# Veason-silverbullet/DIGAT

Measured on AMD Instinct MI355X. Metric: MIND dev impressions scored/sec (AUC match not run), higher is better.
Workload: dtype f32; 1 GPU; MIND-small default: --graph_encoder=DIGAT neighbors=3 hops=2 (N=10, U=67), d=400, graph_depth=3, fp32 dev inference; projection=auto -> fp16x3, N=10, U=67, d=400, graph_depth=3, news_num=65238, parallelism=dp1 (row shards, no data-path collective), ranks_in_process_group=1

## Files before the change

digat_amd/csrc/digat_glue.inc:

```

__global__ void __launch_bounds__(256) build_user_nodes_kernel(const float4* ue, const float4* topic, float4* Xu,
                                                               long B, int H, int C, int d4, const int* group, const uint8_t* rowmask = nullptr) {
    const long per_row = (long)(H + C) * d4;
    const long total = B * per_row;
    for (long i = (long)blockIdx.x * 256 + threadIdx.x; i < total; i += (long)gridDim.x * 256) {
        const long b = i / per_row;
        if (rowmask && rowmask[b] == 0) continue;
        const long rem = i - b * per_row;
        const long hist = (long)H * d4;
        const long src = group ? group[b] : b;
        Xu[i] = rem < hist ? ue[src * hist + rem] : topic[rem - hist];
    }
}

struct UserNodes3 { const float4* hist[3]; const float4* topic[3]; float4* dst[3]; };
__global__ void __launch_bounds__(256) build_user_nodes3_kernel(const UserNodes3 a, long B, int H, int C, int d4) {
    const int pl = blockIdx.y;
    const float4* ue = a.hist[pl];
    const float4* topic = a.topic[pl];
    float4* Xu = a.dst[pl];
    const long per_row = (long)(H + C) * d4;
    const long total = B * per_row;
    const long hist = (long)H * d4;
    for (long i = (long)blockIdx.x * 256 + threadIdx.x; i < total; i += (long)gridDim.x * 256) {
        const long b = i / per_row;
        const long rem = i - b * per_row;
        Xu[i] = rem < hist ? ue[b * hist + rem] : topic[rem - hist];
    }
}

__global__ void __launch_bounds__(256) user_live_flags_kernel(const uint8_t* Au, const uint8_t* cat_mask, const int64_t* cat_idx,
                                                              int B, int U, int H, int C1, uint8_t* flags, int* cnt, int* entries,
                                                              int* hlast, uint8_t* bflags, int* bcnt,
                                                              unsigned* twin = nullptr, uint8_t* tflags = nullptr, int* tcnt = nullptr,
                                                              const uint8_t* rowmask = nullptr) {
    extern __shared__ __attribute__((aligned(16))) unsigned char live_smem[];
    const int lane = threadIdx.x & 63, wave = threadIdx.x >> 6;
    const int b = blockIdx.x * 4 + wave;
    if (b >= B) return;
    if (rowmask && rowmask[b] == 0) return;
    const int uu = U * U;
    unsigned char* Al = live_smem + wave * ((uu + 63) & ~63);
    {
        const uint8_t* Ag = Au + (long)b * uu;
        for (int k0 = 0; k0 < uu; k0 += 64 * 32) {
            uint8_t v[32];
#pragma unroll
            for (int k = 0; k < 32; ++k) v[k] = Ag[min(k0 + k * 64 + lane, uu - 1)];
#pragma unroll
            for (int k = 0; k < 32; ++k) if (k0 + k * 64 + lane < uu) Al[k0 + k * 64 + lane] = v[k];
// ... 45 lines not shown
            if (i < H) {
                const long c = cat_idx[(long)b * H + i];
                live |= !any_cat || (c >= 0 && c < C1 && cat_mask[(long)b * C1 + c] != 0);
            }
            flags[(long)b * U + i] = live ? 1 : 0;
        }
        lv2[h] = live;
        count += __popcll(__ballot(live));
        const unsigned long long hm = __ballot(live && i < H);
        if (hm) last = 64 * h + 64 - __builtin_clzll(hm);
    }
    if (lane == 0) cnt[b] = count;
    if (lane == 0 && hlast) hlast[b] = last;
    if (twin) {
        int before[2] = {0, 0};
        unsigned word[2] = {0xFFFFFF00u | (unsigned)lane, 0xFFFFFF00u | (unsigned)(lane + 64)};
        unsigned long long rem0 = __ballot(lv2[0]), rem1 = __ballot(lv2[1]);
        while (rem0 | rem1) {
            const int hj = rem0 ? 0 : 1, lj = rem0 ? __builtin_ctzll(rem0) : __builtin_ctzll(rem1);
            const unsigned lo0 = (unsigned)__builtin_amdgcn_readlane((int)(unsigned)(hj ? own0[1] : own0[0]), lj);
            const unsigned hi0 = (unsigned)__builtin_amdgcn_readlane((int)(unsigned)((hj ? own0[1] : own0[0]) >> 32), lj);
            const unsigned lo1 = (unsigned)__builtin_amdgcn_readlane((int)(unsigned)(hj ? own1[1] : own1[0]), lj);
            const unsigned hi1 = (unsigned)__builtin_amdgcn_readlane((int)(unsigned)((hj ? own1[1] : own1[0]) >> 32), lj);
            const unsigned long long r0 = ((unsigned long long)hi0 << 32) | lo0, r1 = ((unsigned long long)hi1 << 32) | lo1;
            const bool e0 = lv2[0] && own0[0] == r0 && own1[0] == r1, e1 = lv2[1] && own0[1] == r0 && own1[1] == r1;
            const unsigned long long g0 = __ballot(e0), g1 = __ballot(e1);
            const unsigned long long below = (1ull << lane) - 1ull, above = lane == 63 ? 0ull : ~((2ull << lane) - 1ull);
            if (e0) {
                before[0] = __popcll(g0 & below);
                unsigned long long a0 = g0 & above, a1 = g1;
#pragma unroll
                for (int k = 1; k < TWIN_R; ++k) {
                    int j = -1;
                    if (a0) { j = __builtin_ctzll(a0); a0 &= a0 - 1ull; }
                    else if (a1) { j = 64 + __builtin_ctzll(a1); a1 &= a1 - 1ull; }
                    if (j >= 0) word[0] = (word[0] & ~(0xFFu << (8 * k))) | ((unsigned)j << (8 * k));
                }
            }
            if (e1) {
                before[1] = __popcll(g0) + __popcll(g1 & below);
                unsigned long long a1 = g1 & above;
#pragma unroll
                for (int k = 1; k < TWIN_R; ++k) {
                    if (a1) { const int j = 64 + __builtin_ctzll(a1); a1 &= a1 - 1ull; word[1] = (word[1] & ~(0xFFu << (8 * k))) | ((unsigned)j << (8 * k)); }
                }
            }
            rem0 &= ~g0; rem1 &= ~g1;
        }
        int leads = 0;
#pragma unroll
        for (int h = 0; h < 2; ++h) {
            const int i = lane + 64 * h;
            const bool lead = lv2[h] && (before[h] % TWIN_R) == 0;
            if (i < U) {
                twin[(long)b * U + i] = lead ? word[h] : 0xFFFFFFFFu;
                tflags[(long)b * U + i] = lead ? 1 : 0;
            }
            leads += __popcll(__ballot(lead));
        }
        if (lane == 0) tcnt[b] = leads;
    }
    if (entries && lane == 0) entries[b] = nz + (all_live ? U : 0);
    if (bflags) {
        int bc = 0;
        for (int c0 = 0; c0 < C1; c0 += 64) {
            const int c = c0 + lane;
            const bool bl = c < C1 && (!any_cat || cat_mask[(long)b * C1 + c] != 0);
            if (c < C1) bflags[(long)b * C1 + c] = bl ? 1 : 0;
            bc += __popcll(__ballot(bl));
        }
        if (lane == 0) bcnt[b] = bc;
    }
}

struct LiveExpand {
    const uint8_t* flags_g; const unsigned* twin_g; const uint8_t* tflags_g; const uint8_t* bflags_g;
    const int* cnt_g; const int* entries_g; const int* hlast_g; const int* bcnt_g; const int* tcnt_g;
    uint8_t* flags; unsigned* twin; uint8_t* tflags; uint8_t* bflags;
    int* cnt; int* entries; int* hlast; int* bcnt; int* tcnt;
};
__global__ void __launch_bounds__(256) live_expand_kernel(const LiveExpand a, const int* row_group, int B, int U, int C1) {
    const int lane = threadIdx.x & 63, wave = threadIdx.x >> 6;
    const int b = blockIdx.x * 4 + wave;
    if (b >= B) return;
    const long g = __builtin_amdgcn_readfirstlane(row_group[b]);
    if (a.flags_g == a.flags && g == b) return;
    for (int i = lane; i < U; i += 64) {
        a.flags[(long)b * U + i] = a.flags_g[g * U + i];
        if (a.twin) { a.twin[(long)b * U + i] = a.twin_g[g * U + i]; a.tflags[(long)b * U + i] = a.tflags_g[g * U + i]; }
    }
    if (a.bflags) for (int c = lane; c < C1; c += 64) a.bflags[(long)b * C1 + c] = a.bflags_g[g * C1 + c];
    if (lane == 0) {
        a.cnt[b] = a.cnt_g[g];
        if (a.hlast) a.hlast[b] = a.hlast_g[g];
        if (a.bcnt) a.bcnt[b] = a.bcnt_g[g];
        if (a.tcnt) a.tcnt[b] = a.tcnt_g[g];
        if (a.entries) a.entries[b] = a.entries_g[g];
    }
}

__global__ void __launch_bounds__(1024) sparse_decide_kernel(const int* entries, int B, int n, int per_node, int* flag) {
    __shared__ long long part[16];
    long long s = 0;
    for (int b = threadIdx.x; b < B; b += 1024) s += entries[b];
    for (int o = 32; o > 0; o >>= 1) s += __shfl_xor(s, o, 64);
    if ((threadIdx.x & 63) == 0) part[threadIdx.x >> 6] = s;
    __syncthreads();
    if (threadIdx.x == 0) {
        long long tot = 0;
        for (int w = 0; w < 16; ++w) tot += part[w];
        *flag = tot <= (long long)per_node * B * n ? 1 : 0;
// ... 286 lines not shown
```

digat_amd/csrc/digat_kernels.hip:

```cpp
#include <hip/hip_runtime.h>
#include <stdint.h>
#include <string.h>
#include <stdlib.h>
#include <atomic>
#include <initializer_list>
#include <mutex>
#include <unordered_map>
#include <utility>

#include "../../include/digat_hip.h"

typedef float v4f __attribute__((ext_vector_type(4)));

#define DIGAT_CHECK_LAUNCH()                                   \
    do {                                                       \
        if (hipGetLastError() != hipSuccess) return DIGAT_ERR_LAUNCH; \
    } while (0)

static inline size_t align_up(size_t v, size_t a) { return (v + a - 1) / a * a; }
struct Arena {
    char* base; size_t cap, used; bool ok;
    Arena() : base(nullptr), cap(SIZE_MAX), used(0), ok(true) {}
    Arena(void* p, size_t n) : base((char*)p), cap(n), used(0), ok(p != nullptr) {}
    template <class T> T* take(size_t count) {
// ... 119 lines not shown
__device__ __forceinline__ float leaky02_uniform(float e) {
    const float t = 0.2f * e;
    float r;
    asm("v_max_f32 %0, %1, %2" : "=v"(r) : "s"(e), "v"(t));
    return r;
}
__device__ __forceinline__ unsigned hash32(unsigned x) {
    x ^= x >> 16; x *= 0x7feb352dU; x ^= x >> 15; x *= 0x846ca68bU; x ^= x >> 16;
    return x;
}
__host__ __device__ __forceinline__ unsigned drop_threshold(float p) { return (unsigned)(p * 4294967296.0); }
__device__ __forceinline__ bool drop_keep(unsigned seed, long e, unsigned thr) {
    return hash32((unsigned)e * 0x9E3779B9U + hash32(seed + (unsigned)(e >> 32))) >= thr;
}
constexpr int TWIN_R = DIGAT_TWIN_R;
#include "digat_gemm.inc"
#include "digat_xattn.inc"
#include "digat_context.inc"
#include "digat_ctxfused.inc"
#include "digat_glue.inc"

extern "C" {

int digat_version(void) { return DIGAT_ABI_VERSION; }

const char* digat_error_string(int code) {
    switch (code) {
        case DIGAT_OK: return "ok";
        case DIGAT_ERR_ARG: return "bad argument (null pointer or negative size)";
        case DIGAT_ERR_SHAPE: return "unsupported shape (d % 4 != 0, graph larger than DIGAT_MAX_NODES, depth too large)";
// ... 17 lines not shown
    w.h = a.take<float>(3 * nd);
    if (w.h) { w.P = w.h + nd; w.Q = w.P + nd; }
    w.r = a.take<float>((size_t)B * d);
    w.alpha = a.take<float>((size_t)B * n * n);
    return w;
}
size_t digat_xattn_workspace_bytes(int B, int n, int d) { Arena a; xattn_carve(a, B, n, d); return a.used; }

int digat_xattn_pairwise_fwd(const float* Pr, const float* Q, const float* h, const float* X,
                             const float* a, const uint8_t* A, float* out, float* alpha,
                             int B, int n, int d, void* stream) {
    if (!Pr || !Q || !h || !X || !a || !A || !out || !alpha) return DIGAT_ERR_ARG;
    return launch_xattn_pairwise(Pr, Q, h, X, a, A, out, alpha, B, n, d, (hipStream_t)stream);
}

struct TwinLists { const unsigned* word; const int* list; const int* count; };

struct XattnOpts {
    const void* wsplit = nullptr;
    const int* rowidx = nullptr; const int* nrows_dev = nullptr; const uint8_t* live = nullptr;
    int sparse_mode = DIGAT_XATTN_DENSE; const int* sparse_flag = nullptr;
    int pq_x3 = 0, pq_mode = 0, centre_limit = 0, gemm_format = 0, prof_part = 0;
    unsigned* range_flag = nullptr; const TwinLists* tw = nullptr;
};

static int xattn_core(const float* X, const uint8_t* A, const float* r_given,
                      const float* W, const float* bW, const float* F1, const float* F2, const float* a,
                      float* out, float* alpha_out, int B, int n, int d, void* workspace, size_t workspace_bytes, hipStream_t st,
                      const XattnOpts& o = XattnOpts()) {
    Arena ar(workspace, workspace_bytes);
    const XattnWs w = xattn_carve(ar, B, n, d);
// ... 15 lines not shown
                     d / 4 <= 256 && d % 80 == 0 && (long)B * n >= 2048;
    const long ld8 = (long)align_up((size_t)d + 4 * (size_t)(d / 80), 64);
    if (pq16) { g.bf16_segs = 6; if (pq_mode & 2) g.x1_segs = 6; }
    if (pq8) { g.fp8_segs = 6; g.ldy8 = ld8; if (pq_mode & 2) g.x1_segs = 6; }
    const bool listed = rowidx && gemm_takes_row_list(g);
    if (listed) { g.rowidx = rowidx; g.nrows_dev = nrows_dev; }
    const int rc = launch_gemm(g, st, DIGAT_KERNEL_PROJ);
    if (rc) return rc;
    const int* skip_if = nullptr;
    if (sparse_mode != DIGAT_XATTN_DENSE && !alpha_out && n > 16 && d / 4 <= 256) {
        SparseArgs sg{P, Q, h, X, a, A, out, nullptr, nullptr, listed ? live : nullptr,
                      sparse_mode == DIGAT_XATTN_AUTO ? o.sparse_flag : nullptr, B, n, d / 4, 0, nullptr, nullptr,
                      listed && live ? rowidx : nullptr, listed && live ? nrows_dev : nullptr, 0, nullptr, pq8 ? 2 : (pq16 ? 1 : 0), o.centre_limit};
        sg.ld8 = pq8 ? ld8 : 0;
        sg.prof_part = o.prof_part;
        if (o.tw && listed && live) { sg.twin = o.tw->word; sg.twlist = o.tw->list; sg.twcount = o.tw->count; }
        const int rcs = launch_sparse(sg, st);
        if (rcs || sparse_mode == DIGAT_XATTN_SPARSE) return rcs;
        skip_if = o.sparse_flag;
    }
    return launch_xattn_pairwise(P, Q, h, X, a, A, out, alpha, B, n, d, st, listed ? live : nullptr, nullptr, nullptr,
                                 alpha_out != nullptr, skip_if);
}

static int xattn_fwd_k3(const float* X, const uint8_t* A, const float* ctx, const float* W, const float* bW, const float* F1,
                        const float* F2, const float* F3, const float* b3, const float* a, float* out, float* alpha_out,
                        int B, int n, int d, void* workspace, size_t workspace_bytes, void* stream, const XattnOpts& o = XattnOpts()) {
    Arena ar(workspace, workspace_bytes);
    const XattnWs w = xattn_carve(ar, B, n, d);
    if (!ar.ok) return DIGAT_ERR_WORKSPACE;
    if (B == 0) return DIGAT_OK;
// ... 324 lines not shown
struct FoldCtxWs { float *T, *T2, *glob; };
struct EncoderWs {
    float *Xu[2], *Xn[2];
    char* xws; size_t xws_bytes;
    XattnWs xu;
    char* cws; size_t cws_bytes;
    FoldCtxWs fc;
    float *kq_t, *kq_u, *r_user[2], *r_news;
    char* xws_news; size_t xws_news_bytes;
    XattnWs xn;
    int *cnt, *off, *idx, *cnt2, *off2, *idx2, *entries, *flag, *hlast;
    uint8_t *flags1, *flags2;
    int *cnt_n, *off_n, *idx_n; uint8_t* flags_n;
    int *l0_gs, *l0_off; uint8_t* l0_lead; int* l0_idx;
    unsigned* tw_word; int* tw_list; uint8_t* tw_flags; int *tw_cnt, *tw_off;
    int *gl_off, *gl_idx;
    int* idx32;
    uint8_t *Au, *cm; int64_t* ci;
    uint8_t *fg, *tfg; unsigned* twg; uint8_t* bfg; int *cg, *eg, *hg, *bcg, *tcg;
    uint8_t *same, *is_leader, *lead; int* leader_of;
};
static bool encoder_carve(Arena& a, int B, int N, int H, int C, int d, int variant, EncoderWs& e) {
    const int U = H + C, C1 = C + 1, nmax = N > U ? N : U;
    const size_t b = (size_t)B, bd = b * d, bu = b * U;
    e = EncoderWs();
    for (float*& x : e.Xu) x = a.take<float>(bu * d);
    for (float*& x : e.Xn) x = a.take<float>(b * N * d);
    Arena xa = a.sub(digat_xattn_workspace_bytes(B, nmax, d));
    e.xws = xa.base; e.xws_bytes = xa.cap;
    e.xu = xattn_carve(xa, B, U, d);
    Arena ca = a.sub(max_sz(digat_news_ctx_workspace_bytes(B, N, d), digat_user_ctx_workspace_bytes(B, U, H, C1, d)));
    e.cws = ca.base; e.cws_bytes = ca.cap;
    e.fc = FoldCtxWs{ca.take<float>(b * C1 * d), ca.take<float>(b * C1 * d), ca.take<float>(bd)};
    e.kq_t = a.take<float>(bd); e.kq_u = a.take<float>(bd);
// ... 6 lines not shown
    e.entries = a.take<int>(b); e.flag = a.take<int>(64); e.hlast = a.take<int>(b);
    e.flags1 = a.take<uint8_t>(bu); e.flags2 = a.take<uint8_t>(b * C1);
    e.cnt_n = a.take<int>(b); e.off_n = a.take<int>(b + 1); e.idx_n = a.take<int>(b * N); e.flags_n = a.take<uint8_t>(b * N);
    e.l0_gs = a.take<int>(b + 64); e.l0_off = a.take<int>(b + 64); e.l0_lead = a.take<uint8_t>(b); e.l0_idx = a.take<int>(bu);
    e.tw_word = a.take<unsigned>(bu); e.tw_list = a.take<int>(bu); e.tw_flags = a.take<uint8_t>(bu);
    e.tw_cnt = a.take<int>(b + 64); e.tw_off = a.take<int>(b + 64);
    e.gl_off = a.take<int>(b + 64); e.gl_idx = a.take<int>(bu);
    e.idx32 = a.take<int>(b);
    if (variant == ENC_GROUPED) {
        const size_t g = b / 4 + 1;
        e.Au = a.take<uint8_t>(bu * U); e.cm = a.take<uint8_t>(b * C1); e.ci = a.take<int64_t>(b * H);
        e.fg = a.take<uint8_t>(g * U); e.tfg = a.take<uint8_t>(g * U); e.twg = a.take<unsigned>(g * U); e.bfg = a.take<uint8_t>(g * C1);
        for (int** x : {&e.cg, &e.eg, &e.hg, &e.bcg, &e.tcg}) *x = a.take<int>(g);
    } else if (variant == ENC_SHARED) {
        e.same = a.take<uint8_t>(b); e.is_leader = a.take<uint8_t>(b); e.lead = a.take<uint8_t>(b); e.leader_of = a.take<int>(b);
    }
    return a.ok && xa.ok && ca.ok && na.ok;
}
static size_t encoder_ws_bytes(int B, int N, int H, int C, int d, int variant) { Arena a; EncoderWs e; encoder_carve(a, B, N, H, C, d, variant, e); return a.used; }

struct EncoderCall {
    const digat_params* p;
    const float* Xn_in; const uint8_t *An, *Mn;
    const float* ue;
    const uint8_t *Au, *cat_mask; const int64_t* cat_idx;
    const float* c_n0; float *out_news, *out_user;
    int B, N, H;
    void* workspace; size_t workspace_bytes; hipStream_t st;
    int variant;
    const int* row_group; int G;
// ... 106 lines not shown
    const int pq_mode = ((p->flags & DIGAT_PQ_BF16) ? 1 : 0) | ((p->flags & DIGAT_PQ_X1) ? 2 : 0) | ((p->flags & DIGAT_PQ_FP8) ? 4 : 0);
    const bool want_scan = want_live || sparse_mode == DIGAT_XATTN_AUTO;
    const int* rowidx = nullptr;
    const int* nrows_dev = nullptr;
    uint8_t* live_flags = nullptr;
    const int *pend_rowidx = nullptr, *pend_nrows = nullptr, *pend_bidx = nullptr, *pend_nb = nullptr, *pend_hlast = nullptr;

    uint8_t* pend_flags = nullptr;
    const bool l0_chunked = row_group && (Xg0 || shared) && want_live &&
                            sparse_mode == DIGAT_XATTN_SPARSE && d / 4 <= 128 && U <= 128;
    const uint8_t* const l0_lead = shared ? run_lead : w.l0_lead;
    const bool twins = want_live && sparse_mode == DIGAT_XATTN_SPARSE && d / 4 <= 128 && U <= 128 && L > 1;
    unsigned* const tw_word = w.tw_word; uint8_t* const tw_flags = w.tw_flags;
    int *const tw_list = w.tw_list, *const tw_cnt = w.tw_cnt, *const tw_off = w.tw_off;
    int *const gl_off = w.gl_off, *const gl_idx = w.gl_idx, *const l0_gs = w.l0_gs, *const l0_off = w.l0_off, *const l0_idx = w.l0_idx;
    TwinLists tw_pub{nullptr, nullptr, nullptr};
    auto find_live_rows = [&](hipStream_t sq) -> int {
        int *cnt = w.cnt, *off = w.off, *idx = w.idx, *cnt2 = w.cnt2, *off2 = w.off2, *idx2 = w.idx2, *entries = w.entries, *flag = w.flag;
        int* hlast = w.hlast; uint8_t *flags1 = w.flags1, *flags2 = w.flags2;
        ProfScope prof(DIGAT_KERNEL_GLUE, (double)B * ((double)U * U + 2.0 * C1 + H * 8.0) + (double)B * (U + C1) * 6, sq);
        if (l0_chunked && !shared) {
            hipLaunchKernelGGL(sparse_l0_chunks_kernel, dim3(1), dim3(1024), 0, sq, row_group, B, G, SPARSE_L0_ROWS, l0_gs, w.l0_lead);
            DIGAT_CHECK_LAUNCH();
        }
        if (shared) {
            const bool want_entries = sparse_mode == DIGAT_XATTN_AUTO;
            hipLaunchKernelGGL(user_live_flags_kernel, dim3((B + 3) / 4), dim3(256), (size_t)4 * ((U * U + 63) & ~63), sq, Au, cat_mask, cat_idx, B, U, H, C1,
                               flags1, cnt, want_entries ? entries : (int*)nullptr, hlast, flags2, cnt2,
                               twins ? tw_word : (unsigned*)nullptr, twins ? tw_flags : (uint8_t*)nullptr, twins ? tw_cnt : (int*)nullptr,
                               run_leader);
            DIGAT_CHECK_LAUNCH();
            const LiveExpand le{flags1, twins ? tw_word : nullptr, tw_flags, flags2, cnt, entries, hlast, cnt2, tw_cnt,
                                flags1, twins ? tw_word : nullptr, tw_flags, flags2,
                                cnt, want_entries ? entries : nullptr, hlast, cnt2, twins ? tw_cnt : nullptr};
            hipLaunchKernelGGL(live_expand_kernel, dim3((B + 3) / 4), dim3(256), 0, sq, le, row_group, B, U, C1);
            DIGAT_CHECK_LAUNCH();
        } else if (c.variant == ENC_GROUPED) {
            uint8_t *fg = w.fg, *tfg = w.tfg, *bfg = w.bfg; unsigned* twg = w.twg;
            int *cg = w.cg, *eg = w.eg, *hg = w.hg, *bcg = w.bcg, *tcg = w.tcg;
            const bool want_entries = sparse_mode == DIGAT_XATTN_AUTO;
            hipLaunchKernelGGL(user_live_flags_kernel, dim3((G + 3) / 4), dim3(256), (size_t)4 * ((U * U + 63) & ~63), sq, c.Au_g, c.cm_g, c.ci_g, G, U, H, C1,
                               fg, cg, want_entries ? eg : (int*)nullptr, hg, bfg, bcg,
                               twins ? twg : (unsigned*)nullptr, twins ? tfg : (uint8_t*)nullptr, twins ? tcg : (int*)nullptr);
            DIGAT_CHECK_LAUNCH();
            const LiveExpand le{fg, twins ? twg : nullptr, tfg, bfg, cg, eg, hg, bcg, tcg,
                                flags1, twins ? tw_word : nullptr, tw_flags, flags2,
                                cnt, want_entries ? entries : nullptr, hlast, cnt2, twins ? tw_cnt : nullptr};
            hipLaunchKernelGGL(live_expand_kernel, dim3((B + 3) / 4), dim3(256), 0, sq, le, row_group, B, U, C1);
            DIGAT_CHECK_LAUNCH();
        } else {
            hipLaunchKernelGGL(user_live_flags_kernel, dim3((B + 3) / 4), dim3(256), (size_t)4 * ((U * U + 63) & ~63), sq, Au, cat_mask, cat_idx, B, U, H, C1,
                               flags1, cnt, sparse_mode == DIGAT_XATTN_AUTO ? entries : (int*)nullptr, hlast, flags2, cnt2,
                               twins ? tw_word : (unsigned*)nullptr, twins ? tw_flags : (uint8_t*)nullptr, twins ? tw_cnt : (int*)nullptr);
            DIGAT_CHECK_LAUNCH();
        }
        if (sparse_mode == DIGAT_XATTN_AUTO) {
            hipLaunchKernelGGL(sparse_decide_kernel, dim3(1), dim3(1024), 0, sq, (const int*)entries, B, U, SPARSE_PER_NODE, flag);
            DIGAT_CHECK_LAUNCH();
            sparse_flag = flag;
        }
        ScanPair sp{{cnt, cnt2}, {off, off2}, {nullptr, nullptr}};
        ListPair lp{{flags1, flags2}, {off, off2}, {U, C1, U, U, U, U}, {idx, idx2}, {nullptr, nullptr}};
        int jobs = 2;
        if (l0_chunked) {
            sp.cnt[jobs] = cnt; sp.off[jobs] = l0_off; sp.rowmask[jobs] = l0_lead;
            lp.flags[jobs] = flags1; lp.off[jobs] = l0_off; lp.out[jobs] = l0_idx; lp.rowmask[jobs] = l0_lead;
            ++jobs;
        }
        if (twins) {
            sp.cnt[jobs] = tw_cnt; sp.off[jobs] = tw_off;
            lp.flags[jobs] = tw_flags; lp.off[jobs] = tw_off; lp.out[jobs] = tw_list;
            lp.width[jobs] = U;
            ++jobs;
        }
        if (shared) {
            sp.cnt[jobs] = cnt; sp.off[jobs] = gl_off; sp.rowmask[jobs] = run_leader;
            lp.flags[jobs] = flags1; lp.off[jobs] = gl_off; lp.out[jobs] = gl_idx; lp.rowmask[jobs] = run_leader;
            lp.width[jobs] = U;
            ++jobs;
        }
        hipLaunchKernelGGL(exclusive_scan2_kernel, dim3(jobs), dim3(1024), 0, sq, sp, B);
        DIGAT_CHECK_LAUNCH();
        hipLaunchKernelGGL(live_list2_kernel, dim3((B + 3) / 4, jobs), dim3(256), 0, sq, lp, B);
        DIGAT_CHECK_LAUNCH();
        pend_rowidx = idx; pend_nrows = off + B; pend_bidx = idx2; pend_nb = off2 + B; pend_flags = flags1; pend_hlast = hlast;
        return DIGAT_OK;
    };
    auto publish_live_rows = [&]() {
        rowidx = pend_rowidx; nrows_dev = pend_nrows; bucket_idx = pend_bidx; nbuckets_dev = pend_nb; live_flags = pend_flags;
        hist_last = pend_hlast;
        if (twins) tw_pub = TwinLists{tw_word, tw_list, tw_off + B};
    };
    const int side_mode = (p->flags & DIGAT_PARAMS_SIDE_STREAM_OFF) ? 0 : ((p->flags & DIGAT_PARAMS_SIDE_STREAM_ON) ? 1 : 2);
    SideStream* side = (side_mode == 0 || (side_mode == 2 && B >= 2048)) ? nullptr : side_stream(st);
    const bool news_early = L > 0 && N <= 16 && d / 4 <= 256;
    const bool news_lists_on = L > 0 && d / 4 <= 256 && !(p->flags & DIGAT_PARAMS_NO_LIVE_ROWS);
    const bool news_lists = news_lists_on && ((!news_early && (p->flags & DIGAT_NEWS_XATTN_SPARSE) && N > 16) || (news_early && L > 1 && B >= 2048));
    const int* news_rowidx = nullptr; const int* news_nrows = nullptr; const uint8_t* news_flags = nullptr;
    auto news_project = [&](int layer, const float* Xn_cur, hipStream_t sq) -> int {
        const digat_layer_params& ln = p->news[layer];
        GemmArgs gp = gemm_plain(Xn_cur, d, ln.W, ln.bW, w.xn.h, d, B * N, d, d, 0);
        gp.w[1] = ln.F1; gp.bias[1] = nullptr; gp.y[1] = w.xn.P;
        gp.w[2] = ln.F2; gp.bias[2] = nullptr; gp.y[2] = w.xn.Q;
        gp.nsegs = 3;
        gp.x3_segs = pq_x3 ? 6 : 0;
        gp.m_dispatch = 1 << 30;
// ... 556 lines not shown
```

digat_amd/csrc/digat_xattn.inc:

```

struct ScoreArgs {
    const float* P;
    const float* Q; const float* a; const uint8_t* A; float* alpha;
    float* s_out;
    const uint8_t* live;
    const int* qgroup;
    const float* radd;
    const int64_t* bindex;
    const float* agg_h; const float* agg_x; float* agg_out;
    int B, n, d, d4;
    int NT, SN, CC4, nchunks, RB;
    int img_slots;
    int ring_slots;
    int ninstr;
    int am_off;
    int a_off;
    int tl_off;
    int ld_off;
    int pm_off;
    const int* skip_if;
    uint8_t* amask; float* adrop; float drop_p; unsigned drop_seed;
};
constexpr int XA_RING = 3;
constexpr int XA_KMAX = 4;
// ... 452 lines not shown
    const int* run_if;
    int B, n, d4;
    int xgroup;
    const uint8_t* fill_flags; float* fill_out;
    const int* rowidx; const int* nrows_dev;
    int G;
    unsigned long long* exec_rows;
    int pq16;
    int centre_limit;
    int xcd_group;
    long ld8;
    const unsigned* twin; const int* twlist; const int* twcount;
    unsigned exec_unit;
    int prof_part;
    float* t_alpha; float* t_spre; uint8_t* t_amask; float t_p; unsigned t_seed;
#ifdef DIGAT_SPARSE_TIMERS
    unsigned long long* timers;
#endif
};

#ifdef DIGAT_SPARSE_TIMERS
#define SP_T0() unsigned long long sp_last = __builtin_amdgcn_s_memtime(); const bool sp_on = g.timers && (blockIdx.x & 15) == 0
#define SP_T(k) do { if (sp_on) { asm volatile("s_waitcnt vmcnt(0) lgkmcnt(0)" ::: "memory"); const unsigned long long t__ = __builtin_amdgcn_s_memtime(); \
                     if (lane == 0) atomicAdd(g.timers + (k), t__ - sp_last); sp_last = __builtin_amdgcn_s_memtime(); } } while (0)
#else
#define SP_T0() do {} while (0)
#define SP_T(k) do {} while (0)
#endif

#ifndef DIGAT_SPARSE_NBR
// ... 723 lines not shown
    uint8_t ab0 = g.A[rho * n + min(lane, n - 1)], ab1 = g.A[rho * n + min(lane + 64, n - 1)];
    int rho_next_v = g.twlist[min(k + stride, count - 1)];
    for (;;) {
        const long kn = k + stride;
        const bool more = kn < count;
        const long rho_n = more ? (long)__builtin_amdgcn_readfirstlane(rho_next_v) : rho;
        const unsigned word_n = g.twin[rho_n];
        const uint8_t ab0_n = g.A[rho_n * n + min(lane, n - 1)], ab1_n = g.A[rho_n * n + min(lane + 64, n - 1)];
        rho_next_v = g.twlist[min(kn + stride, count - 1)];
        xattn_sparse_twin_chunk<U, R>(g, rho, (unsigned)__builtin_amdgcn_readfirstlane((int)word_v), ab0, ab1, lane);
        if (!more) break;
        k = kn; rho = rho_n; word_v = word_n; ab0 = ab0_n; ab1 = ab1_n;
    }
}

__global__ void __launch_bounds__(1024) sparse_count_kernel(const int* rowidx, const int* nrows_dev, int n, int limit, unsigned unit, unsigned unit_nbr,
                                                            unsigned long long* out) {
    __shared__ int part[16], part2[16];
    const int total = *nrows_dev;
    int lo = 0, hi = 0;
    for (int k = blockIdx.x * 1024 + threadIdx.x; k < total; k += gridDim.x * 1024) { lo += (rowidx[k] % n) < limit; ++hi; }
    for (int o = 32; o > 0; o >>= 1) { lo += __shfl_xor(lo, o, 64); hi += __shfl_xor(hi, o, 64); }
    if ((threadIdx.x & 63) == 0) { part[threadIdx.x >> 6] = lo; part2[threadIdx.x >> 6] = hi; }
    __syncthreads();
    if (threadIdx.x == 0) {
        long t = 0, m = 0;
        for (int w = 0; w < 16; ++w) { t += part[w]; m += part2[w]; }
        if (m) atomicAdd(out, (unsigned long long)t * unit + (unsigned long long)(m - t) * unit_nbr);
    }
}
// ... 47 lines not shown
    }
    return DIGAT_OK;
}

#ifdef DIGAT_SPARSE_TIMERS
static unsigned long long* g_sparse_timers = nullptr;
extern "C" int digat_debug_sparse_timers(double* out9) {
    if (!g_sparse_timers || !out9) return DIGAT_ERR_ARG;
    unsigned long long h[9];
    if (hipDeviceSynchronize() != hipSuccess || hipMemcpy(h, g_sparse_timers, sizeof(h), hipMemcpyDeviceToHost) != hipSuccess) return DIGAT_ERR_LAUNCH;
    for (int k = 0; k < 9; ++k) out9[k] = (double)h[k];
    (void)hipMemset(g_sparse_timers, 0, 16 * 8);
    return DIGAT_OK;
}
#endif
static int launch_sparse(const SparseArgs& g_in, hipStream_t st) {
    SparseArgs g = g_in;
    if (g.n > 128 || g.d4 > 256) return DIGAT_ERR_SHAPE;
    { const int rcp = sparse_prof_bytes(g, st); if (rcp) return rcp; }
    ProfScope prof(DIGAT_KERNEL_XATTN, sparse_bytes(g), st, 0.0, sparse_part(g));
    unsigned blocks = (unsigned)(((long)g.B * g.n + 3) / 4);
    if (g.run_if && blocks > 2048u) blocks = 2048u;
    constexpr int SPARSE_XCD_GROUP = 16;
    g.xcd_group = SPARSE_XCD_GROUP;
#ifdef DIGAT_SPARSE_TIMERS
    if (!g_sparse_timers && hipMalloc((void**)&g_sparse_timers, 16 * 8) == hipSuccess) (void)hipMemset(g_sparse_timers, 0, 16 * 8);
    g.timers = g.rowidx ? g_sparse_timers : nullptr;
#endif
    blocks = (blocks + 8u * g.xcd_group - 1) / (8u * g.xcd_group) * (8u * g.xcd_group);
    if (g.twin && g.twlist && g.twcount && g.rowidx && !g.pq16 && !g.radd && !g.group && !g.run_if && !g.fill_flags && g.d4 <= 128) {
        constexpr unsigned TWIN_GRID_CAP = 8192;
        if (blocks > TWIN_GRID_CAP) blocks = TWIN_GRID_CAP;
        blocks = (blocks * 4 + DIGAT_TWIN_WPG - 1) / DIGAT_TWIN_WPG;
        if (g.d4 <= 64) hipLaunchKernelGGL((xattn_sparse_twin_kernel<1, TWIN_R>), dim3(blocks), dim3(64 * DIGAT_TWIN_WPG), 0, st, g);
        else hipLaunchKernelGGL((xattn_sparse_twin_kernel<2, TWIN_R>), dim3(blocks), dim3(64 * DIGAT_TWIN_WPG), 0, st, g);
        DIGAT_CHECK_LAUNCH();
        return DIGAT_OK;
    }
    if (g.pq16 == 2) {
        if (g.radd || g.d4 % 20 || g.ld8 < 4 * g.d4 + 4 * (g.d4 / 20) || (g.ld8 & 7)) return DIGAT_ERR_SHAPE;
        if (g.d4 <= 64) hipLaunchKernelGGL((xattn_sparse_kernel<1, 2, false>), dim3(blocks), dim3(256), 0, st, g);
        else if (g.d4 <= 128) hipLaunchKernelGGL((xattn_sparse_kernel<2, 2, false>), dim3(blocks), dim3(256), 0, st, g);
        else hipLaunchKernelGGL((xattn_sparse_kernel<4, 2, false>), dim3(blocks), dim3(256), 0, st, g);
    } else if (g.pq16) {
        if (g.radd || (g.d4 & 1)) return DIGAT_ERR_SHAPE;
        if (g.d4 <= 64) hipLaunchKernelGGL((xattn_sparse_kernel<1, 1, false>), dim3(blocks), dim3(256), 0, st, g);
        else if (g.d4 <= 128) hipLaunchKernelGGL((xattn_sparse_kernel<2, 1, false>), dim3(blocks), dim3(256), 0, st, g);
        else hipLaunchKernelGGL((xattn_sparse_kernel<4, 1, false>), dim3(blocks), dim3(256), 0, st, g);
    } else if (g.radd) {
        if (g.d4 <= 64) hipLaunchKernelGGL((xattn_sparse_kernel<1, 0, true>), dim3(blocks), dim3(256), 0, st, g);
        else if (g.d4 <= 128) hipLaunchKernelGGL((xattn_sparse_kernel<2, 0, true>), dim3(blocks), dim3(256), 0, st, g);
// ... 256 lines not shown
```

Before: 37990 impressions/s.

## Batch same-neighborhood history nodes into classes sharing staged neighbor tiles

```diff
diff --git a/digat_amd/csrc/digat_glue.inc b/digat_amd/csrc/digat_glue.inc
--- a/digat_amd/csrc/digat_glue.inc
+++ b/digat_amd/csrc/digat_glue.inc
@@ -33,7 +33,8 @@
                                                               int B, int U, int H, int C1, uint8_t* flags, int* cnt, int* entries,
                                                               int* hlast, uint8_t* bflags, int* bcnt,
                                                               unsigned* twin = nullptr, uint8_t* tflags = nullptr, int* tcnt = nullptr,
-                                                              const uint8_t* rowmask = nullptr) {
+                                                              const uint8_t* rowmask = nullptr,
+                                                              uint8_t* cflags = nullptr, int* ccnt = nullptr, uint4* cmask = nullptr) {
     extern __shared__ __attribute__((aligned(16))) unsigned char live_smem[];
     const int lane = threadIdx.x & 63, wave = threadIdx.x >> 6;
     const int b = blockIdx.x * 4 + wave;
@@ -109,6 +110,9 @@
     if (lane == 0 && hlast) hlast[b] = last;
     if (twin) {
         int before[2] = {0, 0};
+        bool on_twin[2] = {true, true}, cl_lead[2] = {false, false};
+        const unsigned long long hm0 = H >= 64 ? ~0ull : ((1ull << H) - 1ull);
+        const unsigned long long hm1 = H > 64 ? (H >= 128 ? ~0ull : ((1ull << (H - 64)) - 1ull)) : 0ull;
         unsigned word[2] = {0xFFFFFF00u | (unsigned)lane, 0xFFFFFF00u | (unsigned)(lane + 64)};
         unsigned long long rem0 = __ballot(lv2[0]), rem1 = __ballot(lv2[1]);
         while (rem0 | rem1) {
@@ -120,10 +124,21 @@
             const unsigned long long r0 = ((unsigned long long)hi0 << 32) | lo0, r1 = ((unsigned long long)hi1 << 32) | lo1;
             const bool e0 = lv2[0] && own0[0] == r0 && own1[0] == r1, e1 = lv2[1] && own0[1] == r0 && own1[1] == r1;
             const unsigned long long g0 = __ballot(e0), g1 = __ballot(e1);
+            const unsigned long long gh0 = g0 & hm0, gh1 = g1 & hm1;
+            const bool cls = cflags && __popcll(gh0) + __popcll(gh1) >= CLASS_MIN && __popcll(r0) + __popcll(r1) >= 2;
+            const unsigned long long t0 = cls ? g0 & ~gh0 : g0, t1 = cls ? g1 & ~gh1 : g1;
+            if (cls) {
+                const int il = gh0 ? __builtin_ctzll(gh0) : 64 + __builtin_ctzll(gh1);
+                if (lane == (il & 63)) {
+                    if (il < 64) cl_lead[0] = true; else cl_lead[1] = true;
+                    cmask[(long)b * U + il] = make_uint4((unsigned)gh0, (unsigned)(gh0 >> 32), (unsigned)gh1, (unsigned)(gh1 >> 32));
+                }
+            }
             const unsigned long long below = (1ull << lane) - 1ull, above = lane == 63 ? 0ull : ~((2ull << lane) - 1ull);
             if (e0) {
-                before[0] = __popcll(g0 & below);
-                unsigned long long a0 = g0 & above, a1 = g1;
+                on_twin[0] = (t0 >> lane) & 1ull;
+                before[0] = __popcll(t0 & below);
+                unsigned long long a0 = t0 & above, a1 = t1;
 #pragma unroll
                 for (int k = 1; k < TWIN_R; ++k) {
                     int j = -1;
@@ -133,8 +148,9 @@
                 }
             }
             if (e1) {
-                before[1] = __popcll(g0) + __popcll(g1 & below);
-                unsigned long long a1 = g1 & above;
+                on_twin[1] = (t1 >> lane) & 1ull;
+                before[1] = __popcll(t0) + __popcll(t1 & below);
+                unsigned long long a1 = t1 & above;
 #pragma unroll
                 for (int k = 1; k < TWIN_R; ++k) {
                     if (a1) { const int j = 64 + __builtin_ctzll(a1); a1 &= a1 - 1ull; word[1] = (word[1] & ~(0xFFu << (8 * k))) | ((unsigned)j << (8 * k)); }
@@ -142,18 +158,21 @@
             }
             rem0 &= ~g0; rem1 &= ~g1;
         }
-        int leads = 0;
+        int leads = 0, classes = 0;
 #pragma unroll
         for (int h = 0; h < 2; ++h) {
             const int i = lane + 64 * h;
-            const bool lead = lv2[h] && (before[h] % TWIN_R) == 0;
+            const bool lead = lv2[h] && on_twin[h] && (before[h] % TWIN_R) == 0;
             if (i < U) {
                 twin[(long)b * U + i] = lead ? word[h] : 0xFFFFFFFFu;
                 tflags[(long)b * U + i] = lead ? 1 : 0;
+                if (cflags) cflags[(long)b * U + i] = cl_lead[h] ? 1 : 0;
             }
             leads += __popcll(__ballot(lead));
+            classes += __popcll(__ballot(cl_lead[h]));
         }
         if (lane == 0) tcnt[b] = leads;
+        if (lane == 0 && ccnt) ccnt[b] = classes;
     }
     if (entries && lane == 0) entries[b] = nz + (all_live ? U : 0);
     if (bflags) {
@@ -173,6 +192,7 @@
     const int* cnt_g; const int* entries_g; const int* hlast_g; const int* bcnt_g; const int* tcnt_g;
     uint8_t* flags; unsigned* twin; uint8_t* tflags; uint8_t* bflags;
     int* cnt; int* entries; int* hlast; int* bcnt; int* tcnt;
+    const uint8_t* cflags_g; const uint4* cmask_g; const int* ccnt_g; uint8_t* cflags; uint4* cmask; int* ccnt;
 };
 __global__ void __launch_bounds__(256) live_expand_kernel(const LiveExpand a, const int* row_group, int B, int U, int C1) {
     const int lane = threadIdx.x & 63, wave = threadIdx.x >> 6;
@@ -183,6 +203,11 @@
     for (int i = lane; i < U; i += 64) {
         a.flags[(long)b * U + i] = a.flags_g[g * U + i];
         if (a.twin) { a.twin[(long)b * U + i] = a.twin_g[g * U + i]; a.tflags[(long)b * U + i] = a.tflags_g[g * U + i]; }
+        if (a.twin && a.cflags) {
+            const uint8_t cf = a.cflags_g[g * U + i];
+            a.cflags[(long)b * U + i] = cf;
+            if (cf) a.cmask[(long)b * U + i] = a.cmask_g[g * U + i];
+        }
     }
     if (a.bflags) for (int c = lane; c < C1; c += 64) a.bflags[(long)b * C1 + c] = a.bflags_g[g * C1 + c];
     if (lane == 0) {
@@ -190,6 +215,7 @@
         if (a.hlast) a.hlast[b] = a.hlast_g[g];
         if (a.bcnt) a.bcnt[b] = a.bcnt_g[g];
         if (a.tcnt) a.tcnt[b] = a.tcnt_g[g];
+        if (a.tcnt && a.ccnt) a.ccnt[b] = a.ccnt_g[g];
         if (a.entries) a.entries[b] = a.entries_g[g];
     }
 }
diff --git a/digat_amd/csrc/digat_kernels.hip b/digat_amd/csrc/digat_kernels.hip
--- a/digat_amd/csrc/digat_kernels.hip
+++ b/digat_amd/csrc/digat_kernels.hip
@@ -157,6 +157,7 @@
     return hash32((unsigned)e * 0x9E3779B9U + hash32(seed + (unsigned)(e >> 32))) >= thr;
 }
 constexpr int TWIN_R = DIGAT_TWIN_R;
+constexpr int CLASS_MIN = 3;
 #include "digat_gemm.inc"
 #include "digat_xattn.inc"
 #include "digat_context.inc"
@@ -204,7 +205,8 @@
     return launch_xattn_pairwise(Pr, Q, h, X, a, A, out, alpha, B, n, d, (hipStream_t)stream);
 }
 
-struct TwinLists { const unsigned* word; const int* list; const int* count; };
+struct TwinLists { const unsigned* word; const int* list; const int* count;
+                   const int* clist; const int* ccount; const uint4* cmask; };
 
 struct XattnOpts {
     const void* wsplit = nullptr;
@@ -250,7 +252,10 @@
                       listed && live ? rowidx : nullptr, listed && live ? nrows_dev : nullptr, 0, nullptr, pq8 ? 2 : (pq16 ? 1 : 0), o.centre_limit};
         sg.ld8 = pq8 ? ld8 : 0;
         sg.prof_part = o.prof_part;
-        if (o.tw && listed && live) { sg.twin = o.tw->word; sg.twlist = o.tw->list; sg.twcount = o.tw->count; }
+        if (o.tw && listed && live) {
+            sg.twin = o.tw->word; sg.twlist = o.tw->list; sg.twcount = o.tw->count;
+            sg.cllist = o.tw->clist; sg.clcount = o.tw->ccount; sg.clmask = o.tw->cmask;
+        }
         const int rcs = launch_sparse(sg, st);
         if (rcs || sparse_mode == DIGAT_XATTN_SPARSE) return rcs;
         skip_if = o.sparse_flag;
@@ -605,10 +610,12 @@
     int *cnt_n, *off_n, *idx_n; uint8_t* flags_n;
     int *l0_gs, *l0_off; uint8_t* l0_lead; int* l0_idx;
     unsigned* tw_word; int* tw_list; uint8_t* tw_flags; int *tw_cnt, *tw_off;
+    uint8_t* cl_flags; uint4* cl_mask; int *cl_cnt, *cl_off, *cl_list;
     int *gl_off, *gl_idx;
     int* idx32;
     uint8_t *Au, *cm; int64_t* ci;
     uint8_t *fg, *tfg; unsigned* twg; uint8_t* bfg; int *cg, *eg, *hg, *bcg, *tcg;
+    uint8_t* cfg; uint4* cmg; int* ccg;
     uint8_t *same, *is_leader, *lead; int* leader_of;
 };
 static bool encoder_carve(Arena& a, int B, int N, int H, int C, int d, int variant, EncoderWs& e) {
@@ -645,6 +652,16 @@
         for (int** x : {&e.cg, &e.eg, &e.hg, &e.bcg, &e.tcg}) *x = a.take<int>(g);
     } else if (variant == ENC_SHARED) {
         e.same = a.take<uint8_t>(b); e.is_leader = a.take<uint8_t>(b); e.lead = a.take<uint8_t>(b); e.leader_of = a.take<int>(b);
+    }
+    if (e.xu.alpha) {
+        Arena cl(e.xu.alpha, bu * U * sizeof(float));
+        e.cl_flags = cl.take<uint8_t>(bu); e.cl_mask = cl.take<uint4>(bu); e.cl_cnt = cl.take<int>(b + 64); e.cl_off = cl.take<int>(b + 64);
+        e.cl_list = cl.take<int>(bu);
+        if (variant == ENC_GROUPED) {
+            const size_t g = b / 4 + 1;
+            e.cfg = cl.take<uint8_t>(g * U); e.cmg = cl.take<uint4>(g * U); e.ccg = cl.take<int>(g);
+        }
+        if (!cl.ok) { e.cl_flags = nullptr; e.cfg = nullptr; }
     }
     return a.ok && xa.ok && ca.ok && na.ok;
 }
@@ -781,7 +798,10 @@
     unsigned* const tw_word = w.tw_word; uint8_t* const tw_flags = w.tw_flags;
     int *const tw_list = w.tw_list, *const tw_cnt = w.tw_cnt, *const tw_off = w.tw_off;
     int *const gl_off = w.gl_off, *const gl_idx = w.gl_idx, *const l0_gs = w.l0_gs, *const l0_off = w.l0_off, *const l0_idx = w.l0_idx;
-    TwinLists tw_pub{nullptr, nullptr, nullptr};
+    const bool classes = twins && w.cl_flags != nullptr;
+    uint8_t* const cl_flags = w.cl_flags; uint4* const cl_mask = w.cl_mask;
+    int *const cl_cnt = w.cl_cnt, *const cl_off = w.cl_off, *const cl_list = w.cl_list;
+    TwinLists tw_pub{nullptr, nullptr, nullptr, nullptr, nullptr, nullptr};
     auto find_live_rows = [&](hipStream_t sq) -> int {
         int *cnt = w.cnt, *off = w.off, *idx = w.idx, *cnt2 = w.cnt2, *off2 = w.off2, *idx2 = w.idx2, *entries = w.entries, *flag = w.flag;
         int* hlast = w.hlast; uint8_t *flags1 = w.flags1, *flags2 = w.flags2;
@@ -795,11 +815,12 @@
             hipLaunchKernelGGL(user_live_flags_kernel, dim3((B + 3) / 4), dim3(256), (size_t)4 * ((U * U + 63) & ~63), sq, Au, cat_mask, cat_idx, B, U, H, C1,
                                flags1, cnt, want_entries ? entries : (int*)nullptr, hlast, flags2, cnt2,
                                twins ? tw_word : (unsigned*)nullptr, twins ? tw_flags : (uint8_t*)nullptr, twins ? tw_cnt : (int*)nullptr,
-                               run_leader);
+                               run_leader, classes ? cl_flags : (uint8_t*)nullptr, classes ? cl_cnt : (int*)nullptr, classes ? cl_mask : (uint4*)nullptr);
             DIGAT_CHECK_LAUNCH();
             const LiveExpand le{flags1, twins ? tw_word : nullptr, tw_flags, flags2, cnt, entries, hlast, cnt2, tw_cnt,
                                 flags1, twins ? tw_word : nullptr, tw_flags, flags2,
-                                cnt, want_entries ? entries : nullptr, hlast, cnt2, twins ? tw_cnt : nullptr};
+                                cnt, want_entries ? entries : nullptr, hlast, cnt2, twins ? tw_cnt : nullptr,
+                                cl_flags, cl_mask, cl_cnt, classes ? cl_flags : nullptr, cl_mask, cl_cnt};
             hipLaunchKernelGGL(live_expand_kernel, dim3((B + 3) / 4), dim3(256), 0, sq, le, row_group, B, U, C1);
             DIGAT_CHECK_LAUNCH();
         } else if (c.variant == ENC_GROUPED) {
@@ -808,17 +829,20 @@
             const bool want_entries = sparse_mode == DIGAT_XATTN_AUTO;
             hipLaunchKernelGGL(user_live_flags_kernel, dim3((G + 3) / 4), dim3(256), (size_t)4 * ((U * U + 63) & ~63), sq, c.Au_g, c.cm_g, c.ci_g, G, U, H, C1,
                                fg, cg, want_entries ? eg : (int*)nullptr, hg, bfg, bcg,
-                               twins ? twg : (unsigned*)nullptr, twins ? tfg : (uint8_t*)nullptr, twins ? tcg : (int*)nullptr);
+                               twins ? twg : (unsigned*)nullptr, twins ? tfg : (uint8_t*)nullptr, twins ? tcg : (int*)nullptr,
+                               nullptr, classes ? w.cfg : (uint8_t*)nullptr, classes ? w.ccg : (int*)nullptr, classes ? w.cmg : (uint4*)nullptr);
             DIGAT_CHECK_LAUNCH();
             const LiveExpand le{fg, twins ? twg : nullptr, tfg, bfg, cg, eg, hg, bcg, tcg,
                                 flags1, twins ? tw_word : nullptr, tw_flags, flags2,
-                                cnt, want_entries ? entries : nullptr, hlast, cnt2, twins ? tw_cnt : nullptr};
+                                cnt, want_entries ? entries : nullptr, hlast, cnt2, twins ? tw_cnt : nullptr,
+                                w.cfg, w.cmg, w.ccg, classes ? cl_flags : nullptr, cl_mask, cl_cnt};
             hipLaunchKernelGGL(live_expand_kernel, dim3((B + 3) / 4), dim3(256), 0, sq, le, row_group, B, U, C1);
             DIGAT_CHECK_LAUNCH();
         } else {
             hipLaunchKernelGGL(user_live_flags_kernel, dim3((B + 3) / 4), dim3(256), (size_t)4 * ((U * U + 63) & ~63), sq, Au, cat_mask, cat_idx, B, U, H, C1,
                                flags1, cnt, sparse_mode == DIGAT_XATTN_AUTO ? entries : (int*)nullptr, hlast, flags2, cnt2,
-                               twins ? tw_word : (unsigned*)nullptr, twins ? tw_flags : (uint8_t*)nullptr, twins ? tw_cnt : (int*)nullptr);
+                               twins ? tw_word : (unsigned*)nullptr, twins ? tw_flags : (uint8_t*)nullptr, twins ? tw_cnt : (int*)nullptr,
+                               nullptr, classes ? cl_flags : (uint8_t*)nullptr, classes ? cl_cnt : (int*)nullptr, classes ? cl_mask : (uint4*)nullptr);
             DIGAT_CHECK_LAUNCH();
         }
         if (sparse_mode == DIGAT_XATTN_AUTO) {
@@ -837,6 +861,12 @@
         if (twins) {
             sp.cnt[jobs] = tw_cnt; sp.off[jobs] = tw_off;
             lp.flags[jobs] = tw_flags; lp.off[jobs] = tw_off; lp.out[jobs] = tw_list;
+            lp.width[jobs] = U;
+            ++jobs;
+        }
+        if (classes) {
+            sp.cnt[jobs] = cl_cnt; sp.off[jobs] = cl_off;
+            lp.flags[jobs] = cl_flags; lp.off[jobs] = cl_off; lp.out[jobs] = cl_list;
             lp.width[jobs] = U;
             ++jobs;
         }
@@ -856,7 +886,7 @@
     auto publish_live_rows = [&]() {
         rowidx = pend_rowidx; nrows_dev = pend_nrows; bucket_idx = pend_bidx; nbuckets_dev = pend_nb; live_flags = pend_flags;
         hist_last = pend_hlast;
-        if (twins) tw_pub = TwinLists{tw_word, tw_list, tw_off + B};
+        if (twins) tw_pub = TwinLists{tw_word, tw_list, tw_off + B, classes ? cl_list : nullptr, classes ? cl_off + B : nullptr, classes ? cl_mask : nullptr};
     };
     const int side_mode = (p->flags & DIGAT_PARAMS_SIDE_STREAM_OFF) ? 0 : ((p->flags & DIGAT_PARAMS_SIDE_STREAM_ON) ? 1 : 2);
     SideStream* side = (side_mode == 0 || (side_mode == 2 && B >= 2048)) ? nullptr : side_stream(st);
diff --git a/digat_amd/csrc/digat_xattn.inc b/digat_amd/csrc/digat_xattn.inc
--- a/digat_amd/csrc/digat_xattn.inc
+++ b/digat_amd/csrc/digat_xattn.inc
@@ -490,6 +490,7 @@
     unsigned exec_unit;
     int prof_part;
     float* t_alpha; float* t_spre; uint8_t* t_amask; float t_p; unsigned t_seed;
+    const int* cllist; const int* clcount; const uint4* clmask;
 #ifdef DIGAT_SPARSE_TIMERS
     unsigned long long* timers;
 #endif
@@ -1243,6 +1244,208 @@
     }
 }
 
+constexpr int CLASS_BLK = 8;
+template <int U>
+__global__ void __launch_bounds__(256, U <= 2 ? 5 : 1) xattn_sparse_twin_class_kernel(const SparseArgs g) {
+    extern __shared__ __attribute__((aligned(16))) unsigned char smem[];
+    constexpr int R = 2, BLK = CLASS_BLK;
+    const int lane = threadIdx.x & 63, wave = __builtin_amdgcn_readfirstlane(threadIdx.x >> 6);
+    const int n = g.n, d4 = g.d4;
+    float4* Ps = reinterpret_cast<float4*>(smem);
+    float4* Hs = Ps + BLK * d4;
+    const long count = *g.clcount;
+    if ((long)blockIdx.x >= count) return;
+    const float4* a4 = reinterpret_cast<const float4*>(g.a);
+    float4 av[U];
+    unsigned c4l[U];
+#pragma unroll
+    for (int u = 0; u < U; ++u) {
+        const int c4 = min(lane + 64 * u, d4 - 1);
+        c4l[u] = (unsigned)c4;
+        const float4 aa = a4[c4];
+        av[u] = lane + 64 * u < d4 ? aa : f4_zero();
+    }
+    typedef unsigned long long u64;
+    auto lowest = [](u64 s0, u64 s1) -> int { return s0 ? __builtin_ctzll(s0) : 64 + __builtin_ctzll(s1); };
+    auto drop = [](u64& s0, u64& s1, int k) { for (int i = 0; i < k && (s0 | s1); ++i) { if (s0) s0 &= s0 - 1ull; else s1 &= s1 - 1ull; } };
+    auto nth = [&](u64 s0, u64 s1, int k) -> int {
+        const int first = lowest(s0, s1);
+        drop(s0, s1, k);
+        return (s0 | s1) ? lowest(s0, s1) : first;
+    };
+    for (long k = blockIdx.x; k < count; k += gridDim.x) {
+        const long rho = __builtin_amdgcn_readfirstlane(g.cllist[k]);
+        const long b = rho / n;
+        const uint4 mk = g.clmask[rho];
+        const uint8_t ab0 = g.A[rho * n + min(lane, n - 1)], ab1 = g.A[rho * n + min(lane + 64, n - 1)];
+        u64 M0 = ((u64)(unsigned)__builtin_amdgcn_readfirstlane((int)mk.y) << 32) | (unsigned)__builtin_amdgcn_readfirstlane((int)mk.x);
+        u64 M1 = ((u64)(unsigned)__builtin_amdgcn_readfirstlane((int)mk.w) << 32) | (unsigned)__builtin_amdgcn_readfirstlane((int)mk.z);
+        if (g.centre_limit > 0) {
+            const int lim = g.centre_limit;
+            M0 &= lim >= 64 ? ~0ull : ((1ull << lim) - 1ull);
+            M1 &= lim > 64 ? (lim >= 128 ? ~0ull : ((1ull << (lim - 64)) - 1ull)) : 0ull;
+        }
+        const u64 A0 = __ballot(lane < n && ab0 != 0), A1 = __ballot(lane + 64 < n && ab1 != 0);
+        const int deg = __popcll(A0) + __popcll(A1);
+        if (deg < 2) continue;
+        const bool one = deg <= BLK;
+        const float4* Pb = reinterpret_cast<const float4*>(g.P) + b * n * d4;
+        const float4* Hb = reinterpret_cast<const float4*>(g.h) + b * n * d4;
+        while (M0 | M1) {
+            const int cm = min(BLK, __popcll(M0) + __popcll(M1));
+            const int nr = (wave < cm ? 1 : 0) + (wave + 4 < cm ? 1 : 0);
+            int mem[R];
+            mem[0] = nth(M0, M1, wave);
+            mem[1] = nr > 1 ? nth(M0, M1, wave + 4) : mem[0];
+            drop(M0, M1, BLK);
+            float4 q[R][U];
+#pragma unroll
+            for (int r = 0; r < R; ++r)
+#pragma unroll
+                for (int u = 0; u < U; ++u) q[r][u] = reinterpret_cast<const float4*>(g.Q)[(b * n + mem[r]) * d4 + c4l[u]];
+            float sc[R][2];
+#pragma unroll
+            for (int r = 0; r < R; ++r) { sc[r][0] = -INFINITY; sc[r][1] = -INFINITY; }
+            {
+                u64 m0 = A0, m1 = A1;
+                while (m0 | m1) {
+                    const int js[2] = {nth(m0, m1, wave), nth(m0, m1, wave + 4)};
+                    v4f lp[2][U], lh[2][U];
+#pragma unroll
+                    for (int s = 0; s < 2; ++s)
+#pragma unroll
+                        for (int u = 0; u < U; ++u) lp[s][u] = *reinterpret_cast<const v4f*>(Pb + (long)js[s] * d4 + c4l[u]);
+                    if (one) {
+#pragma unroll
+                        for (int s = 0; s < 2; ++s)
+#pragma unroll
+                            for (int u = 0; u < U; ++u) lh[s][u] = *reinterpret_cast<const v4f*>(Hb + (long)js[s] * d4 + c4l[u]);
+                    }
+                    __syncthreads();
+#pragma unroll
+                    for (int s = 0; s < 2; ++s)
+#pragma unroll
+                        for (int u = 0; u < U; ++u)
+                            if (lane + 64 * u < d4) {
+                                *reinterpret_cast<v4f*>(Ps + (wave + 4 * s) * d4 + lane + 64 * u) = lp[s][u];
+                                if (one) *reinterpret_cast<v4f*>(Hs + (wave + 4 * s) * d4 + lane + 64 * u) = lh[s][u];
+                            }
+                    __syncthreads();
+                    const float4* Pt = Ps;
+#pragma unroll 1
+                    for (int t = 0; t < BLK && (m0 | m1); ++t, Pt += d4) {
+                        const int jt = lowest(m0, m1);
+                        drop(m0, m1, 1);
+                        float4 p[U];
+#pragma unroll
+                        for (int u = 0; u < U; ++u) p[u] = Pt[c4l[u]];
+#pragma unroll
+                        for (int r = 0; r < R; ++r) {
+                            if (r < nr) {
+                                float part = 0.f;
+#pragma unroll
+                                for (int u = 0; u < U; ++u) {
+                                    const float4 pk = p[u];
+                                    part = fmaf(av[u].x, fmaxf(pk.x + q[r][u].x, 0.f), part);
+                                    part = fmaf(av[u].y, fmaxf(pk.y + q[r][u].y, 0.f), part);
+                                    part = fmaf(av[u].z, fmaxf(pk.z + q[r][u].z, 0.f), part);
+                                    part = fmaf(av[u].w, fmaxf(pk.w + q[r][u].w, 0.f), part);
+                                }
+                                const float e = wave_sum(part);
+                                const float lk = leaky02_uniform(e);
+                                if (lane == (jt & 63)) { if (jt < 64) sc[r][0] = lk; else sc[r][1] = lk; }
+                            }
+                        }
+                    }
+                }
+            }
+            float al[R][2];
+#pragma unroll
+            for (int r = 0; r < R; ++r) {
+                const float mx = wave_max(fmaxf(sc[r][0], sc[r][1]));
+                const float e0 = sc[r][0] > -INFINITY ? expf(sc[r][0] - mx) : 0.f;
+                const float e1 = sc[r][1] > -INFINITY ? expf(sc[r][1] - mx) : 0.f;
+                const float inv = wave_sum(e0 + e1);
+                al[r][0] = e0 / inv;
+                al[r][1] = e1 / inv;
+            }
+            float4 xin[R][U];
+            {
+                unsigned xo[U];
+#pragma unroll
+                for (int u = 0; u < U; ++u) { xo[u] = c4l[u]; asm volatile("" : "+v"(xo[u]) : "v"(al[0][0])); }
+#pragma unroll
+                for (int u = 0; u < U; ++u) xin[0][u] = reinterpret_cast<const float4*>(g.X)[(b * n + mem[0]) * d4 + xo[u]];
+            }
+            float4 acc[R][U];
+#pragma unroll
+            for (int r = 0; r < R; ++r)
+#pragma unroll
+                for (int u = 0; u < U; ++u) acc[r][u] = f4_zero();
+            {
+                u64 m0 = A0, m1 = A1;
+                while (m0 | m1) {
+                    if (!one) {
+                        const int js[2] = {nth(m0, m1, wave), nth(m0, m1, wave + 4)};
+                        v4f lh[2][U];
+#pragma unroll
+                        for (int s = 0; s < 2; ++s)
+#pragma unroll
+                            for (int u = 0; u < U; ++u) lh[s][u] = *reinterpret_cast<const v4f*>(Hb + (long)js[s] * d4 + c4l[u]);
+                        __syncthreads();
+#pragma unroll
+                        for (int s = 0; s < 2; ++s)
+#pragma unroll
+                            for (int u = 0; u < U; ++u)
+                                if (lane + 64 * u < d4) *reinterpret_cast<v4f*>(Hs + (wave + 4 * s) * d4 + lane + 64 * u) = lh[s][u];
+                        __syncthreads();
+                    }
+                    const float4* Ht = Hs;
+#pragma unroll 1
+                    for (int t = 0; t < BLK && (m0 | m1); ++t, Ht += d4) {
+                        const int jt = lowest(m0, m1);
+                        drop(m0, m1, 1);
+                        float4 hv[U];
+#pragma unroll
+                        for (int u = 0; u < U; ++u) hv[u] = Ht[c4l[u]];
+#pragma unroll
+                        for (int r = 0; r < R; ++r) {
+                            if (r < nr) {
+                                const float w = jt < 64 ? lane_bcast(al[r][0], jt) : lane_bcast(al[r][1], jt - 64);
+#pragma unroll
+                                for (int u = 0; u < U; ++u) {
+                                    acc[r][u].x = fmaf(w, hv[u].x, acc[r][u].x); acc[r][u].y = fmaf(w, hv[u].y, acc[r][u].y);
+                                    acc[r][u].z = fmaf(w, hv[u].z, acc[r][u].z); acc[r][u].w = fmaf(w, hv[u].w, acc[r][u].w);
+                                }
+                            }
+                        }
+                    }
+                }
+            }
+            if (nr > 1) {
+#pragma unroll
+                for (int u = 0; u < U; ++u) xin[1][u] = reinterpret_cast<const float4*>(g.X)[(b * n + mem[1]) * d4 + c4l[u]];
+            }
+#pragma unroll
+            for (int r = 0; r < R; ++r) {
+                if (r < nr) {
+                    float4* Oi = reinterpret_cast<float4*>(g.out) + (b * n + mem[r]) * d4;
+#pragma unroll
+                    for (int u = 0; u < U; ++u) {
+                        const int c4 = lane + 64 * u;
+                        if (c4 < d4) {
+                            const float4 x = xin[r][u];
+                            const float4 o = make_float4(fmaxf(acc[r][u].x, 0.f) + x.x, fmaxf(acc[r][u].y, 0.f) + x.y,
+                                                         fmaxf(acc[r][u].z, 0.f) + x.z, fmaxf(acc[r][u].w, 0.f) + x.w);
+                            Oi[c4] = o;
+                        }
+                    }
+                }
+            }
+        }
+    }
+}
+
 __global__ void __launch_bounds__(1024) sparse_count_kernel(const int* rowidx, const int* nrows_dev, int n, int limit, unsigned unit, unsigned unit_nbr,
                                                             unsigned long long* out) {
     __shared__ int part[16], part2[16];
@@ -1320,6 +1523,20 @@
     return DIGAT_OK;
 }
 #endif
+static int launch_sparse_class(const SparseArgs& g_in, hipStream_t st) {
+    SparseArgs g = g_in;
+    g.exec_rows = nullptr; g.exec_unit = 0;
+    ProfScope prof(DIGAT_KERNEL_XATTN, (double)g.d4 * 16, st, 0.0, sparse_part(g));
+    constexpr long CLASS_GRID_CAP = 8192;
+    long blocks = ((long)g.B * g.n + 15) / 16;
+    if (blocks > CLASS_GRID_CAP) blocks = CLASS_GRID_CAP;
+    const size_t lds = (size_t)2 * CLASS_BLK * g.d4 * 16;
+    if (g.d4 <= 64) hipLaunchKernelGGL((xattn_sparse_twin_class_kernel<1>), dim3((unsigned)blocks), dim3(256), lds, st, g);
+    else hipLaunchKernelGGL((xattn_sparse_twin_class_kernel<2>), dim3((unsigned)blocks), dim3(256), lds, st, g);
+    DIGAT_CHECK_LAUNCH();
+    return DIGAT_OK;
+}
+
 static int launch_sparse(const SparseArgs& g_in, hipStream_t st) {
     SparseArgs g = g_in;
     if (g.n > 128 || g.d4 > 256) return DIGAT_ERR_SHAPE;
@@ -1341,6 +1558,7 @@
         if (g.d4 <= 64) hipLaunchKernelGGL((xattn_sparse_twin_kernel<1, TWIN_R>), dim3(blocks), dim3(64 * DIGAT_TWIN_WPG), 0, st, g);
         else hipLaunchKernelGGL((xattn_sparse_twin_kernel<2, TWIN_R>), dim3(blocks), dim3(64 * DIGAT_TWIN_WPG), 0, st, g);
         DIGAT_CHECK_LAUNCH();
+        if (g.cllist && g.clcount && g.clmask) return launch_sparse_class(g, st);
         return DIGAT_OK;
     }
     if (g.pq16 == 2) {
```

Result: slower. 36590 impressions/s (-3.7%).
